# populationgenomics/cuKING

Measured on AMD Instinct MI355X. Metric: sample-pairs/s (all-pairs KING), higher is better.
Workload: dtype fp4 products, f32 accumulate (exact integers)

## Files before the change

### cuking_amd/csrc/king_abi.hip

```cpp
#include <hip/hip_runtime.h>

#include <algorithm>
#include <cstdio>
#include <cstdlib>
#include <cstring>
#include <vector>

#include "king_common.h"
#include "king_host.h"
#include "king_kin_summary.h"

using namespace cuking;

namespace {

#define HIP_TRY(expr)                                                      \
  do {                                                                     \
    const hipError_t _e = (expr);                                          \
    if (_e != hipSuccess) {                                                \
      (void)hipGetLastError();  \
      return cuking_fail(_e == hipErrorOutOfMemory ? CUKING_ERR_OUT_OF_MEMORY     \
                                            : CUKING_ERR_DEVICE,           \
                  "%s failed: %s", #expr, hipGetErrorString(_e));          \
    }                                                                      \
// ... 47 lines not shown
  }
};

}

struct cuking_ctx {
  int device = 0;
  cuking_kernel kernel = CUKING_KERNEL_TILED;
  int variant = 0;
  uint32_t band_rows = 0;
  int counts_mode = -1;
  int xcd_swizzle = 2;
  uint32_t dyn_tail_tiles = 16384;

  uint4 *planes = nullptr;
  size_t planes_bytes = 0;
  uint64_t *band_prefix = nullptr;
  size_t band_prefix_bytes = 0;
  TileSpace prefix_for = {0, 0, 0, 0};

  uint32_t split_wgs = 0;
  struct StreamScratch {
    hipStream_t stream;
    uint32_t *split = nullptr;
    uint8_t *filter = nullptr;
    uint64_t filter_tiles = 0;
  };
  std::vector<StreamScratch> scratch;
  unsigned long long filter_totals_retired[kNumTotals] = {};
  uint32_t filter_quadrant_cap = kFilterQuadrantCap;
  uint32_t filter_cand_cap = kFilterCandCap;
  uint32_t filter_split_min_steps = 8;
  int filter_check0 = 1, filter_check1 = 1, filter_check_emit = (int)kCheckEmitCap;
  int filter_rotate = 1;
  uint32_t filter_rotate_min_steps = 128;
  uint32_t filter_rotate_min_tiles = 2048;
  int filter_sort = 1;
  bool filter_lazy_codes = true;
  void *sort_temp = nullptr;
  size_t sort_temp_bytes = 0;

  void *synth_tables = nullptr;
  size_t synth_tables_bytes = 0;
  hipStream_t synth_stream = nullptr;
  hipEvent_t synth_done = nullptr;

  struct Prepared {
    bool valid = false;
    cuking_submatrix sm = {0, 0, 0, 0};
    uint32_t words_per_sample = 0;
    int variant = -1;
    uint32_t tile = 0;
    const uint64_t *bits = nullptr;
    bool codes = true;
    bool dense_order = false;
    std::vector<uint8_t> tiles;
    hipStream_t ordered_on = nullptr;
    bool ordered_valid = false;
  } prepared;
  std::vector<std::pair<hipStream_t, hipEvent_t>> readers;

  bool reuse_prepared = false;
  uint64_t workspace_allocations = 0, host_syncs = 0, conversions_skipped = 0;

  bool timing = false;
  Timer king_timer, prepare_timer;
// ... 142 lines not shown
                       mfma_split_scratch_bytes(ctx->split_wgs), 0,
                       mfma_split_counter_bytes(ctx->split_wgs), stream);
    if (st != CUKING_OK) return st;
  }
  const FilterScratchLayout want = filter_scratch_layout(tiles);
  if (filter && e->filter != nullptr && filter_scratch_layout(e->filter_tiles).bytes < want.bytes) {
    ++ctx->host_syncs;
    HIP_TRY(hipStreamSynchronize(stream));
    free_filter_scratch(ctx, *e);
  }
  if (filter && e->filter == nullptr) {
    st = alloc_scratch(ctx, reinterpret_cast<void **>(&e->filter), want.bytes, want.totals,
                       kFilterCtrlBytes + kFilterTicketBytes, stream);
    if (st != CUKING_OK) return st;
    e->filter_tiles = tiles;
  }
  *out = e;
  return CUKING_OK;
}

bool filter_runs(const cuking_ctx *ctx, uint32_t words_per_sample, bool full, float kin_threshold) {
  return effective_variant(ctx, words_per_sample) == kMfmaFilterVariant && !full &&
         kin_threshold > 0.f && kin_threshold < 0.5f;
}

LaunchSwitches launch_switches(const cuking_ctx *ctx, uint32_t words_per_sample, bool full,
                               float kin_threshold) {
  LaunchSwitches sw;
  sw.xcd_swizzle = (uint32_t)ctx->xcd_swizzle;
  sw.dyn_tail_tiles = ctx->dyn_tail_tiles;
  sw.check0 = (uint32_t)ctx->filter_check0;
  sw.check1 = (uint32_t)ctx->filter_check1;
  sw.check_emit = (uint32_t)ctx->filter_check_emit;
  sw.rotate = (uint32_t)ctx->filter_rotate;
  sw.rotate_min_tiles = ctx->filter_rotate_min_tiles;
  sw.split_min_steps = ctx->filter_split_min_steps;
  sw.filter_runs = filter_runs(ctx, words_per_sample, full, kin_threshold);
  return sw;
}

struct Outputs {
  uint32_t max_results;
  cuking_result *results;
  uint32_t *result_index, *result_overflow;
  cuking_counts *counts;
  float *kin;
  uint64_t kin_ld;
  uint32_t kin_flags;
  uint64_t *sum_hist, *sum_best;
  cuking_kin_bins sum_bins;
  uint32_t *rel_counts;
  uint32_t rel_num;
  float rel_thr[CUKING_REL_THRESHOLDS_MAX];
};
cuking_status launch_args(cuking_ctx *ctx, hipStream_t stream, const cuking_submatrix &sm,
                          uint32_t words_per_sample, const uint64_t *d_bit_sets,
                          const PlaneGeometry &geo, const TileSpace &tiles,
                          uint64_t block_tiles, float kin_threshold, const Outputs &out,
                          TiledArgs *args) {
  TiledArgs &a = *args;
  a = {};
  a.planes = ctx->planes;
  a.geo = geo;
  a.tiles = tiles;
  a.band_prefix = ctx->band_prefix;
  a.i_begin = sm.i_begin;
// ... 358 lines not shown
  const char *key;
  int64_t lo, hi;
  const char *error;
  uint32_t error_arg;
  uint8_t effects;
  int64_t (*get)(const cuking_ctx *);
  void (*set)(cuking_ctx *, int64_t);
  int64_t hole = INT64_MIN;
};

#define CTX_FIELD(f)                                                     \
  [](const cuking_ctx *c) -> int64_t { return (int64_t)c->f; },          \
  [](cuking_ctx *c, int64_t v) { c->f = (decltype(c->f))v; }

const Option kOptions[] = {
    {"variant", 0, kNumTiledVariants - 1, "variant outside [0, %u)", kNumTiledVariants, 0,
     CTX_FIELD(variant)},
    {"band_rows", 0, 64, "band_rows outside [0, 64]", 0, 0, CTX_FIELD(band_rows)},
    {"counts_mode", -1, 1, "counts_mode outside [-1, 1]", 0, 0, CTX_FIELD(counts_mode)},
    {"split_wgs", 0, 4096, "split_wgs outside [0, 4096]", 0, kResizesSlabs, CTX_FIELD(split_wgs)},
    {"xcd_swizzle", 0, 2, "xcd_swizzle outside [0, 2]", 0, 0, CTX_FIELD(xcd_swizzle)},
    {"dyn_tail_tiles", 0, 0x7FFFFFFF, "dyn_tail_tiles outside [0, 2^31)", 0, 0,
     CTX_FIELD(dyn_tail_tiles)},
    {"reuse_prepared", 0, 1, "reuse_prepared outside [0, 1]", 0, 0, CTX_FIELD(reuse_prepared)},
    {"filter_sort", 0, 2, "filter_sort outside [0, 2]", 0, kInvalidatesLayout,
     CTX_FIELD(filter_sort)},
    {"filter_lazy_codes", 0, 1, "filter_lazy_codes outside [0, 1]", 0, kInvalidatesLayout,
     CTX_FIELD(filter_lazy_codes)},
    {"filter_check0", 0, 2, "filter_check0 outside [0, 2]", 0, 0, CTX_FIELD(filter_check0)},
    {"filter_check1", 0, 1 + kNumCheckShares, "filter_check1 outside {0, 1, 3 .. %u}",
     1 + kNumCheckShares, 0, CTX_FIELD(filter_check1), 2},
    {"filter_check_emit", 0, 255, "filter_check_emit outside [0, 255]", 0, 0,
     CTX_FIELD(filter_check_emit)},
    {"filter_rotate", 0, 2 + kNumPhases, "filter_rotate outside [0, %u]", 2 + kNumPhases, 0,
     CTX_FIELD(filter_rotate)},
    {"filter_rotate_min_steps", 1, 1 << 20, "filter_rotate_min_steps outside [1, 2^20]", 0, 0,
     CTX_FIELD(filter_rotate_min_steps)},
    {"filter_rotate_min_tiles", 0, 1 << 30, "filter_rotate_min_tiles outside [0, 2^30]", 0, 0,
     CTX_FIELD(filter_rotate_min_tiles)},
    {"filter_quadrant_cap", 0, 16384, "filter_quadrant_cap outside [0, 16384]", 0, 0,
     CTX_FIELD(filter_quadrant_cap)},
    {"filter_cand_cap", 0, kFilterCandCap, "filter_cand_cap outside [0, %u]", kFilterCandCap, 0,
     CTX_FIELD(filter_cand_cap)},
    {"filter_split_min_steps", 1, 4096, "filter_split_min_steps outside [1, 4096]", 0, 0,
     CTX_FIELD(filter_split_min_steps)},
    {"max_launch_blocks", 0, INT64_MAX, "negative block cap", 0, 0,
     [](const cuking_ctx *) -> int64_t { return (int64_t)max_blocks_override(); },
     [](cuking_ctx *, int64_t v) { set_max_blocks_per_launch((uint64_t)v); }},
    {"filter_check_min_steps", 4, 1 << 20, "filter_check_min_steps outside [4, 2^20]", 0,
     kInvalidatesLayout,
     [](const cuking_ctx *) -> int64_t { return filter_check_min_steps(); },
     [](cuking_ctx *, int64_t v) { set_filter_check_min_steps((uint32_t)v); }},
};
#undef CTX_FIELD

const Option *find_option(const char *key) {
  for (const Option &o : kOptions)
    if (strcmp(o.key, key) == 0) return &o;
  return nullptr;
}

cuking_status read_diagnostic(const cuking_ctx *ctx, const char *key, int64_t *value) {
  const std::pair<const char *, uint64_t> counters[] = {
      {"workspace_allocations", ctx->workspace_allocations},
      {"host_syncs", ctx->host_syncs},
      {"conversions_skipped", ctx->conversions_skipped}};
  for (const auto &c : counters)
    if (strcmp(c.first, key) == 0) {
      *value = (int64_t)c.second;
      return CUKING_OK;
    }
  const char *const totals[kNumTotals] = {"filter_candidates", "filter_dense_quadrants",
                                          "filter_early_exits", "filter_rotated_tiles"};
  static_assert(kTotalCand == 0 && kTotalDense == 1 && kTotalEarly == 2 && kTotalRotated == 3,
                "totals[] in the order of the running totals");
  uint32_t word = 0;
  while (word < kNumTotals && strcmp(totals[word], key) != 0) ++word;
  const bool ticks = strcmp(key, "filter_step_ticks16") == 0;
  if (word == kNumTotals && !ticks)
    return cuking_fail(CUKING_ERR_INVALID_ARGUMENT, "unknown option %s", key);
  if (hipSetDevice(ctx->device) != hipSuccess || hipDeviceSynchronize() != hipSuccess)
    return cuking_fail(CUKING_ERR_DEVICE, "device wait failed");
  unsigned long long sum = 0;
  uint64_t count = 0;
  for (const auto &e : ctx->scratch) {
    if (e.filter == nullptr) continue;
    if (ticks) {
      uint32_t w[8];
      if (hipMemcpy(w, e.filter + kCtrlStepTicks * 4, sizeof w, hipMemcpyDeviceToHost) != hipSuccess)
        return cuking_fail(CUKING_ERR_DEVICE, "reading the filter counters failed");
      for (uint32_t v : w)
        if (v != 0) {
          sum += v;
          ++count;
        }
    } else {
      unsigned long long v = 0;
      if (hipMemcpy(&v, e.filter + filter_scratch_layout(e.filter_tiles).totals + word * 8, 8,
                    hipMemcpyDeviceToHost) != hipSuccess)
        return cuking_fail(CUKING_ERR_DEVICE, "reading the filter counters failed");
      sum += v;
    }
  }
  if (ticks) *value = count != 0 ? (int64_t)(sum / count) : 0;
  else *value = (int64_t)(sum + ctx->filter_totals_retired[word]);
  return CUKING_OK;
}
// ... 877 lines not shown
```

### cuking_amd/csrc/king_common.h

```cpp
#ifndef CUKING_AMD_KING_COMMON_H_
#define CUKING_AMD_KING_COMMON_H_

#include <hip/hip_runtime.h>
#include <stdint.h>

#include "cuking_amd.h"
#include "king_launch_plan.h"
#include "king_submatrix.h"

namespace cuking {

constexpr uint32_t kLayoutWord = 0;
constexpr uint32_t kLayoutQuad = 1;
constexpr uint32_t kLayoutNibble = 2;
constexpr uint32_t kLayoutNibbleStats = 3;

struct PlaneGeometry {
  uint32_t num_rows, num_cols;
  uint32_t rows_padded, cols_padded;
  uint32_t col_base;
  uint32_t s_stride;
  uint32_t k_words;
  uint32_t diag;
};
// ... 76 lines not shown
  uint32_t dense_cap;
  uint32_t fsplit_parts, fsplit_first, fsplit_tile0;
  float4 *fsplit_slabs;
  uint32_t *fsplit_tickets;
  const uint32_t *check_steps;
  const float *prefix_u;
  const unsigned long long *cohort_sums;
  uint32_t check0, check1;
  uint32_t rotate, rotate_min_steps;
  uint32_t rotate_min_tiles;
  uint8_t *tile_done;
  const uint32_t *gate;
  uint32_t gate_count;
  const uint8_t *skip_tiles;
  uint64_t skip_base;
  const uint32_t *perm;
  uint32_t *codes_ready;
  float *dense_kin;
  uint64_t kin_ld;
  uint32_t kin_diag;
  unsigned long long *sum_hist, *sum_best;
  float sum_lo, sum_scale;
  uint32_t sum_bins;
  uint32_t *rel_counts;
  uint32_t rel_num;
  float rel_thr[CUKING_REL_THRESHOLDS_MAX];
};

constexpr uint32_t kCheckEmitCap = 64;
constexpr uint32_t kNumCheckShares = 8;
constexpr uint32_t kCheckShares64[kNumCheckShares] = {8, 50, 53, 56, 58, 60, 61, 62};
constexpr uint32_t kNumPhases = 128;
constexpr uint32_t kPhasesPerShare = kNumPhases / 64;
constexpr uint32_t kNumCum = kNumPhases - 1;
__host__ __device__ inline uint32_t phase_step(uint32_t all_steps, uint32_t x) {
  return (uint32_t)((uint64_t)all_steps * x / kNumPhases);
}
__host__ __device__ inline uint32_t check_step_of(uint32_t all_steps, uint32_t k,
                                                  uint32_t min_steps = 64) {
  if (all_steps < min_steps) return 0;
  return phase_step(all_steps, kCheckShares64[k] * kPhasesPerShare);
}
constexpr uint32_t kFilterSplitSlabs = 256;
constexpr size_t kFilterSlabBytes = 256 * 256 * sizeof(float);
constexpr size_t kFilterTicketBytes = kFilterSplitSlabs * sizeof(uint32_t);
__host__ __device__ inline size_t plane_bytes(const PlaneGeometry &g,
                                              uint32_t layout) {
  const size_t base = (size_t)g.k_words * g.s_stride * (layout == kLayoutQuad ? 8 : 16);
  if (layout == kLayoutNibble) return base + base / 4;
  if (layout == kLayoutNibbleStats)
    return base + base / 4 + base / 2 + (size_t)g.s_stride * sizeof(float2) +
           (size_t)g.s_stride * kNumCum * sizeof(float) + 64 + 64 +
           64 + (size_t)g.s_stride * (4 + 8 + 4 * (kNumCum + 1) + 16);
  return base;
}
__host__ __device__ inline const uint4 *plane_t2(const uint4 *planes, const PlaneGeometry &g) {
  return planes + (size_t)g.k_words * g.s_stride * 5 / 4;
}
__host__ __device__ inline const float2 *plane_stats(const uint4 *planes, const PlaneGeometry &g) {
  return reinterpret_cast<const float2 *>(planes + (size_t)g.k_words * g.s_stride * 7 / 4);
}
__host__ __device__ inline const float *plane_prefix_u(const uint4 *planes, const PlaneGeometry &g) {
  return reinterpret_cast<const float *>(plane_stats(planes, g) + g.s_stride);
}
__host__ __device__ inline const unsigned long long *plane_cohort_sums(const uint4 *planes,
                                                                       const PlaneGeometry &g) {
  return reinterpret_cast<const unsigned long long *>(plane_prefix_u(planes, g) +
                                                      (size_t)g.s_stride * kNumCum);
}

struct TiledVariant {
  const char *name;
  uint32_t tile;
  uint32_t k_chunk;
  uint32_t threads;
  uint32_t lds_bytes;
  uint32_t layout;
};

constexpr uint32_t kMfmaMaxSites = 1u << 24;

constexpr int kNumTiledVariants = 8;
constexpr int kMfmaVariant = 5;
constexpr int kMfmaN4Variant = 6;
constexpr uint32_t kMfmaN4MaxSites = 1u << 22;
static_assert(4ull * kMfmaN4MaxSites <= (1ull << 24), "filter kernel: exact float sums");
constexpr int kMfmaN4Stages = 5;
constexpr uint32_t kMfmaN4LdsBytes = kMfmaN4Stages * 2 * 2 * 4 * 128 * 16;
static_assert(kMfmaN4LdsBytes <= 160 * 1024, "LDS of one CU");
constexpr int kMfmaFilterVariant = 7;
constexpr uint32_t kFilterTile = 256;
constexpr uint32_t kFilterLdsBytes = 5 * 2 * 2 * 2 * 256 * 16;
static_assert(kFilterLdsBytes <= 160 * 1024, "LDS of one CU");
constexpr uint32_t kFilterChunkTiles = 1u << 17;
constexpr uint32_t kFilterCandCap = 1u << 25;
constexpr uint32_t kFilterQuadrantCap = 384;
constexpr size_t kFilterCtrlBytes = 256;
constexpr uint32_t kCtrlCand = 0, kCtrlDense = 1, kCtrlDyn = 2, kCtrlFinished = 3,
                   kCtrlLeft = 4, kCtrlAllLeave = 5, kCtrlGate = 6;
constexpr uint32_t kCtrlStepTicks = 8, kCtrlPos = 16, kPosSlots = 16;
constexpr size_t kCtrlChunkBytes = (kCtrlPos + 8 * kPosSlots * 2) * 4;
constexpr uint32_t kTotalCand = 0, kTotalDense = 1, kTotalEarly = 2, kTotalRotated = 3;
constexpr uint32_t kNumTotals = 4;
__host__ __device__ inline const uint32_t *plane_check_steps(const uint4 *planes,
                                                             const PlaneGeometry &g) {
  return reinterpret_cast<const uint32_t *>(plane_cohort_sums(planes, g) + 8);
}
__host__ __device__ inline uint32_t *plane_flags(const uint4 *planes, const PlaneGeometry &g) {
  return const_cast<uint32_t *>(plane_check_steps(planes, g)) + 16;
}
__host__ __device__ inline uint32_t *plane_perm(const uint4 *planes, const PlaneGeometry &g) {
  return plane_flags(planes, g) + 16;
}
__host__ __device__ inline float2 *plane_tmp_stats(const uint4 *planes, const PlaneGeometry &g) {
  return reinterpret_cast<float2 *>(plane_perm(planes, g) + g.s_stride);
}
__host__ __device__ inline float *plane_tmp_prefix(const uint4 *planes, const PlaneGeometry &g) {
  return reinterpret_cast<float *>(plane_tmp_stats(planes, g) + g.s_stride);
}
__host__ __device__ inline uint32_t *plane_sort_words(const uint4 *planes, const PlaneGeometry &g) {
  return reinterpret_cast<uint32_t *>(plane_tmp_prefix(planes, g) +
                                      (size_t)g.s_stride * (kNumCum + 1));
}
constexpr uint32_t kNoSample = 0xFFFFFFFFu;

struct FilterScratchLayout {
  size_t tile_done, totals, tickets, cand, dense, slabs, bytes;
  uint32_t chunk_tiles, cand_entries;
};
inline FilterScratchLayout filter_scratch_layout(uint64_t tiles) {
  FilterScratchLayout l;
  l.chunk_tiles = (uint32_t)(tiles < kFilterChunkTiles ? (tiles ? tiles : 1) : kFilterChunkTiles);
  const uint64_t cand = (uint64_t)l.chunk_tiles * 4 * 64;
  l.cand_entries = (uint32_t)(cand < kFilterCandCap ? cand : kFilterCandCap);
  auto up = [](size_t x) { return (x + 255) / 256 * 256; };
  l.tile_done = kCtrlChunkBytes;
// ... 98 lines not shown
```

### cuking_amd/csrc/king_filter.hip

```cpp
#include <hip/hip_runtime.h>
#include <stdio.h>

#include <atomic>
#include <stdlib.h>

#include "king_common.h"
#include "king_device.h"
#include "king_kin_summary.h"

#pragma clang diagnostic ignored "-Winline-asm"

namespace cuking {

namespace {

typedef int v8i __attribute__((ext_vector_type(8)));
typedef float v16f __attribute__((ext_vector_type(16)));

constexpr int kT = (int)kFilterTile;
constexpr int kUnits = 2;
constexpr int kStages = 5;
constexpr int kSliceU4 = kT;
constexpr int kStageU4 = 2 * 2 * kUnits * kSliceU4;
constexpr int kStageReqs = 4 * kUnits;
// ... 143 lines not shown
  if (a.dyn_tiles != 0 && wg >= a.launch_tiles) {
    uint32_t *slot = reinterpret_cast<uint32_t *>(lds);
    if (threadIdx.x == 0) *slot = relaxed_add(a.filter_ctrl + kCtrlDyn, 1u);
    __syncthreads();
    const uint32_t next = __builtin_amdgcn_readfirstlane(*slot);
    __syncthreads();
    if (next >= a.dyn_tiles) return false;
    bid = a.launch_tiles + next;
  } else if (a.xcd_chunk == 1) {
    bid = xcd_patch_tile(bid);
    if (bid >= a.launch_tiles) return false;
  }
  t->bid = __builtin_amdgcn_readfirstlane(bid);
  uint32_t tr, tc;
  if (!decode_tile_space(a, a.tile_begin + t->bid, &tr, &tc)) return false;
  t->tr = __builtin_amdgcn_readfirstlane(tr);
  t->tc = __builtin_amdgcn_readfirstlane(tc);
  return true;
}

__device__ __forceinline__ bool launch_verdict(const TiledArgs &a, const uint32_t wg,
                                               uint4 *const lds, uint32_t *xcd_pos) {
  uint32_t *verdict = reinterpret_cast<uint32_t *>(lds);
  if (threadIdx.x == 0) {
    uint32_t leave = relaxed_load(a.filter_ctrl + kCtrlAllLeave);
    auto all_leave = [&] {
      leave = 1;
      relaxed_store(a.filter_ctrl + kCtrlAllLeave, 1u);
      relaxed_store(a.filter_ctrl + kCtrlGate, 1u);
    };
    float mean, sigma;
    if (leave == 0 && a.cohort_sums != nullptr && a.check_steps != nullptr &&
        bound_level(a.cohort_sums, 32.f * (float)a.geo.k_words, &mean, &sigma) &&
        mean - 4.f * sigma > a.kin_threshold && (a.check1 >> 16) != 0)
      all_leave();
    if (leave == 0) {
      const uint32_t dense_so_far =
          relaxed_load(a.filter_ctrl + kCtrlDense) + relaxed_load(a.filter_ctrl + kCtrlLeft);
      const uint32_t finished = relaxed_load(a.filter_ctrl + kCtrlFinished);
      if (finished >= 512 && 2 * dense_so_far > finished) all_leave();
    }
    verdict[0] = leave;
  }
  if (a.rotate == 1 && threadIdx.x < kPosSlots) {
    const uint32_t x = wg & 7;
    const unsigned long long said = relaxed_load(
        reinterpret_cast<const unsigned long long *>(a.filter_ctrl + kCtrlPos) + x * kPosSlots +
        threadIdx.x);
    const uint32_t ticks16 = relaxed_load(a.filter_ctrl + kCtrlStepTicks + x);
    uint32_t pos = (uint32_t)(said >> 32);
    const uint32_t ago = (uint32_t)__builtin_amdgcn_s_memrealtime() - (uint32_t)said;
    if (said != 0 && ticks16 != 0 && ago < 16384u)
      pos += ago * 16u / ticks16;
    verdict[1 + threadIdx.x] = pos;
  }
  __syncthreads();
  const bool give_up = verdict[0] != 0;
  uint32_t pos = 0;
  if (a.rotate == 1) {
#pragma unroll
    for (uint32_t k = 0; k < kPosSlots; ++k) pos = max(pos, verdict[1 + k]);
  }
  *xcd_pos = __builtin_amdgcn_readfirstlane(pos);
  __syncthreads();
  if (give_up && threadIdx.x == 0) relaxed_add(a.filter_totals + kTotalDense, 4ull);
  return give_up;
}

struct CheckPlan {
  uint32_t chk0, chk1;
  uint32_t share1;
  uint32_t phase;
  uint32_t k0;
  uint32_t wrap;
  uint32_t start_abs;
};
__device__ __forceinline__ CheckPlan plan_checks(const TiledArgs &a, const Tile &t,
                                                 const uint32_t xcd_pos, const uint32_t all_steps,
                                                 const uint32_t num_steps) {
  uint32_t chk0 = 0, chk1 = 0, entry1 = 0, share1 = 0;
  uint32_t phase = 0, k0 = 0, wrap = 0, start_abs = 0;
  if (!t.split && a.check_steps != nullptr && a.tile_done != nullptr) {
    if (a.rotate != 0 && all_steps >= a.rotate_min_steps) {
      uint32_t base = 0;
      if (a.rotate == 1) {
        const uint32_t r = xcd_pos % all_steps;
        base = xcd_pos - r;
        phase = (r * kNumPhases + all_steps / 2) / all_steps;
        if (phase >= kNumPhases) {
          phase = 0;
          base += all_steps;
        }
      } else if (a.rotate == 2) {
        phase = (t.bid * 37u + 11u) & (kNumPhases - 1);
      } else {
        phase = (a.rotate - 3u) & (kNumPhases - 1);
      }
      k0 = phase_step(all_steps, phase);
      start_abs = base + k0;
      wrap = k0 != 0 ? all_steps - k0 : 0u;
    }
    float kappa = -1.f, mean, sigma;
    if (bound_level(a.cohort_sums, 256.f * (float)all_steps, &mean, &sigma))
      kappa = mean + 4.6f * sigma + 0.003f;
    auto steps_of = [&](uint32_t share) {
      const uint32_t hi = phase + share * kPhasesPerShare;
      return hi <= kNumPhases ? phase_step(all_steps, hi) - k0
                              : (all_steps - k0) + phase_step(all_steps, hi - kNumPhases);
    };
    if ((a.check0 == 2 || (a.check0 == 1 && kappa > 0.7f * a.kin_threshold)) &&
        a.check_steps[0] != 0)
      chk0 = steps_of(kCheckShares64[0]);
    const uint32_t sw1 = a.check1 & 0xFFu;
    if (sw1 >= 2) {
      entry1 = sw1 - 2;
    } else if (sw1 == 1 && kappa >= 0.f) {
      const float f64 = 64.f * (1.f - 2.f * a.kin_threshold) / (1.f - 2.f * kappa);
      if (f64 <= 62.f) {
        share1 = (uint32_t)ceilf(f64);
        if (share1 < 32) share1 = 32;
        entry1 = 1;
      }
    }
#pragma unroll
    for (uint32_t k = 1; k < kNumCheckShares; ++k)
      if (sw1 >= 2 && k == entry1) share1 = kCheckShares64[k];
    if (share1 != 0 && a.check_steps[entry1] != 0) chk1 = steps_of(share1);
    if (chk0 >= num_steps) chk0 = 0;
    if (chk1 >= num_steps || chk1 <= chk0) chk1 = 0;
  }
  auto sgpr = [](uint32_t v) { return (uint32_t)__builtin_amdgcn_readfirstlane(v); };
  return CheckPlan{sgpr(chk0), sgpr(chk1), sgpr(share1), sgpr(phase), sgpr(k0), sgpr(wrap), sgpr(start_abs)};
}

__device__ __forceinline__ float prefix_u_of(const TiledArgs &a, const CheckPlan &p,
                                             uint32_t share, size_t idx, float total) {
  const uint32_t s_stride = a.geo.s_stride;
  const uint32_t hi = p.phase + share * kPhasesPerShare;
  float u = hi >= kNumPhases ? total
            : hi != 0        ? a.prefix_u[(size_t)(hi - 1) * s_stride + idx]
                             : 0.f;
  if (p.phase != 0) u -= a.prefix_u[(size_t)(p.phase - 1) * s_stride + idx];
  if (hi > kNumPhases) u += a.prefix_u[(size_t)(hi - kNumPhases - 1) * s_stride + idx];
  return u;
}

__device__ __forceinline__ const float2 *stage_bounds(const TiledArgs &a, const Tile &t,
                                                      const CheckPlan &p, uint4 *const lds,
                                                      const bool prefix, const uint32_t share,
                                                      const float thr, const float scale) {
  float2 *const rows = reinterpret_cast<float2 *>(lds), *const cols = rows + kT;
  const float tt = 2.f - 4.f * thr;
  const size_t ir = (size_t)t.tr * kT + threadIdx.x;
  const size_t ic = (size_t)a.geo.col_base + (size_t)t.tc * kT + threadIdx.x;
  float2 r = a.sample_stats[ir], c = a.sample_stats[ic];
  if (prefix) {
    r.x = prefix_u_of(a, p, share, ir, r.x);
    c.x = prefix_u_of(a, p, share, ic, c.x);
  }
  r.y = scale * fmaf(tt, r.y, 8.f);
  c.y = scale * fmaf(tt, c.y, 8.f);
  rows[threadIdx.x] = r;
  cols[threadIdx.x] = c;
  __syncthreads();
  return rows;
}

enum Leave : uint32_t { kStays = 0, kLeftForecast, kLeftEmpty, kLeftEmit };

__device__ __forceinline__ Leave check_sweep(const TiledArgs &a, const Tile &t, const CheckPlan &p,
                                             const v16f (&acc)[4][4], uint4 *const lds,
                                             const bool forecast, const uint32_t all_steps) {
  const Lanes l = lanes_of_thread();
  const float scale = forecast ? (float)kCheckShares64[0] * (1.f / 64.f) : 1.f;
  const uint32_t share = forecast ? kCheckShares64[0] : p.share1;
  const float thr_f = forecast ? a.kin_threshold + 3.66f * rsqrtf(256.f * (float)all_steps)
                               : a.kin_threshold;
  const float2 *const ck_rows = stage_bounds(a, t, p, lds, true, share, thr_f, scale);
  const float2 *const ck_cols = ck_rows + kT;
  uint32_t *const ck_words = reinterpret_cast<uint32_t *>(lds) + 4 * kT;
  const uint32_t emit_cap = (a.check1 >> 8) & 0xFFu;
  uint32_t cnt = 0;
  {
    float2 cc[4];
#pragma unroll
    for (int bj = 0; bj < 4; ++bj) cc[bj] = ck_cols[l.wx * 128 + bj * 32 + l.lr];
#pragma unroll
    for (int bi = 0; bi < 4; ++bi)
#pragma unroll
      for (int r = 0; r < 16; ++r) {
        const float2 cr = ck_rows[l.wy * 128 + bi * 32 + c_row(r, l.g)];
#pragma unroll
        for (int bj = 0; bj < 4; ++bj)
          cnt += fmaf(-8.f, acc[bi][bj][r], cr.x) + cc[bj].x < fminf(cr.y, cc[bj].y) ? 1u : 0u;
      }
  }
#pragma unroll
  for (int off = 32; off > 0; off >>= 1) cnt += __shfl_xor(cnt, off);
  if (l.lane == 0)
    ck_words[l.wave] = forecast ? (cnt > 2 * a.quadrant_cap ? 1u : 0u)
                                : (cnt > emit_cap ? emit_cap + 1 : cnt);
  __syncthreads();
  uint32_t found = forecast ? ck_words[0] + ck_words[1] + ck_words[2] + ck_words[3]
                            : max(max(ck_words[0], ck_words[1]), max(ck_words[2], ck_words[3]));
  found = __builtin_amdgcn_readfirstlane(found);
  __syncthreads();
  if (forecast) return found >= 3 ? kLeftForecast : kStays;
  return found > emit_cap ? kStays : found != 0 ? kLeftEmit : kLeftEmpty;
}

__device__ __forceinline__ bool leave_early(const TiledArgs &a, const Tile &t, const CheckPlan &p,
                                            const Leave left) {
  if (left == kLeftEmit && threadIdx.x == 0) relaxed_add(a.filter_totals + kTotalEarly, 1ull);
  if (p.phase != 0 && threadIdx.x == 0) relaxed_add(a.filter_totals + kTotalRotated, 1ull);
  if (left == kLeftForecast || left == kLeftEmpty) {
    if (threadIdx.x == 0) {
      relaxed_add(a.filter_ctrl + kCtrlFinished, 4u);
      if (left == kLeftForecast) {
        relaxed_add(a.filter_ctrl + kCtrlLeft, 4u);
        relaxed_store(a.filter_ctrl + kCtrlGate, 1u);
        relaxed_add(a.filter_totals + kTotalDense, 4ull);
      } else {
        a.tile_done[t.bid] = 1;
        relaxed_add(a.filter_totals + kTotalEarly, 1ull);
      }
    }
    return true;
  }
  if (!t.split && a.tile_done != nullptr && threadIdx.x == 0) a.tile_done[t.bid] = 1;
  return false;
}

__device__ __forceinline__ bool reduce_pieces(const TiledArgs &a, const Tile &t, v16f (&acc)[4][4],
                                              uint4 *const lds) {
  typedef uint32_t v4u __attribute__((ext_vector_type(4)));
  constexpr uint32_t kSlabU4 = 64 * 256;
  {
    const __amdgpu_buffer_rsrc_t rsrc = __builtin_amdgcn_make_buffer_rsrc(
        a.fsplit_slabs + (size_t)t.piece * kSlabU4, 0, (int)(kSlabU4 * 16), 0x00020000);
#pragma unroll
    for (int bi = 0; bi < 4; ++bi)
#pragma unroll
      for (int bj = 0; bj < 4; ++bj)
#pragma unroll
        for (int r4 = 0; r4 < 4; ++r4) {
          const v16f &c = acc[bi][bj];
// ... 14 lines not shown
    if (last) {
      __builtin_amdgcn_fence(__ATOMIC_ACQUIRE, "agent");
      asm volatile("s_waitcnt vmcnt(0)" ::: "memory");
      *counter = 0;
    }
    *flag = last ? 1u : 0u;
  }
  __syncthreads();
  const bool last = *flag != 0;
  __syncthreads();
  if (!last) return false;
  const uint32_t first_piece = t.piece - t.part;
  for (uint32_t p = 0; p < a.fsplit_parts; ++p) {
    if (p == t.part) continue;
    const float4 *src = a.fsplit_slabs + (size_t)(first_piece + p) * kSlabU4 + threadIdx.x;
#pragma unroll
    for (int bi = 0; bi < 4; ++bi)
#pragma unroll
      for (int bj = 0; bj < 4; ++bj)
#pragma unroll
        for (int r4 = 0; r4 < 4; ++r4) {
          const float4 v = src[((bi * 4 + bj) * 4 + r4) * 256];
          acc[bi][bj][4 * r4] += v.x;
          acc[bi][bj][4 * r4 + 1] += v.y;
          acc[bi][bj][4 * r4 + 2] += v.z;
          acc[bi][bj][4 * r4 + 3] += v.w;
        }
  }
  return true;
}

__device__ __forceinline__ void emit_candidates(const TiledArgs &a, const Tile &t,
                                                const CheckPlan &p, const v16f (&acc)[4][4],
                                                uint4 *const lds, const bool on_prefix) {
  const Lanes l = lanes_of_thread();
  const float2 *const st_rows = stage_bounds(a, t, p, lds, on_prefix, p.share1, a.kin_threshold, 1.f);
  const float2 *const st_cols = st_rows + kT;
  float2 sc[4];
#pragma unroll
  for (int bj = 0; bj < 4; ++bj) sc[bj] = st_cols[l.wx * 128 + bj * 32 + l.lr];

  {
    float best = -1.f;
#pragma unroll
    for (int bi = 0; bi < 4; ++bi)
#pragma unroll
      for (int r = 0; r < 16; ++r) {
        const float2 sr = st_rows[l.wy * 128 + bi * 32 + c_row(r, l.g)];
#pragma unroll
        for (int bj = 0; bj < 4; ++bj)
          best = fmaxf(best, fminf(sr.y, sc[bj].y) -
                                 (fmaf(-8.f, acc[bi][bj][r], sr.x) + sc[bj].x));
      }
    if (l.lane == 0) relaxed_add(a.filter_ctrl + kCtrlFinished, 1u);
    if (__ballot(best > 0.f) == 0) return;
  }

  uint32_t total = 0, base = 0, run = 0;
#pragma nounroll
  for (int pass = 0; pass < 2; ++pass) {
    uint32_t tr_p = t.tr, tc_p = t.tc;
    asm volatile("" : "+s"(tr_p), "+s"(tc_p));
#pragma unroll
    for (int bi = 0; bi < 4; ++bi) {
#pragma unroll
      for (int r = 0; r < 16; ++r) {
        const uint32_t row = l.wy * 128 + bi * 32 + c_row(r, l.g);
        const float2 sr = st_rows[row];
        const uint32_t li = tr_p * kT + row;
// ... 158 lines not shown
    const uint32_t t16_ = (STEPS) >= 32 ? (now_ - t_start) * 16u / (STEPS) : 0u; \
    const uint32_t zero_ = 0;                                                  \
    unsigned long long save_;                                                  \
    asm volatile("s_mov_b64 %0, exec\n\t"                                      \
                 "s_mov_b64 exec, 1\n\t"                                       \
                 "global_store_dwordx2 %1, %2, %3\n\t"                         \
                 "s_mov_b64 exec, %0"                                          \
                 : "=&s"(save_)                                                \
                 : "v"(zero_), "v"(val_), "s"(pos_word)                        \
                 : "memory");                                                  \
    if (t16_ != 0)                                                             \
      asm volatile("s_mov_b64 %0, exec\n\t"                                    \
                   "s_mov_b64 exec, 1\n\t"                                     \
                   "global_store_dword %1, %2, %3\n\t"                         \
                   "s_mov_b64 exec, %0"                                        \
                   : "=&s"(save_)                                              \
                   : "v"(zero_), "v"(t16_), "s"(ticks_word)                    \
                   : "memory");                                                \
  }

__device__ __forceinline__ void filter_tile(const TiledArgs &a, const uint32_t wg, uint4 *const lds) {
  Tile tile;
  if (!take_tile(a, wg, lds, &tile)) return;
  const Lanes ln = lanes_of_thread();
  uint32_t xcd_pos = 0;
  if (!tile.split && a.tile_done != nullptr && launch_verdict(a, wg, lds, &xcd_pos)) return;
  const uint32_t all_steps = a.geo.k_words / (4 * kUnits);
  const uint32_t k_first = __builtin_amdgcn_readfirstlane(
      tile.split ? tile.part * all_steps / a.fsplit_parts : 0u);
  const uint32_t num_steps = __builtin_amdgcn_readfirstlane(
      tile.split ? (tile.part + 1) * all_steps / a.fsplit_parts - k_first : all_steps);
  const CheckPlan plan = plan_checks(a, tile, xcd_pos, all_steps, num_steps);

  const uint32_t wave = ln.wave, chk0 = plan.chk0, chk1 = plan.chk1;
  const uint32_t k0 = plan.k0, wrap = plan.wrap, start_abs = plan.start_abs;
  uint32_t lane16 = ln.lane * 16;
  const uint32_t s_stride = a.geo.s_stride;
  const uint4 *g_rows = a.t2 + (uint64_t)tile.tr * kT;
  const uint4 *g_cols = a.t2 + a.geo.col_base + (uint64_t)tile.tc * kT;

  uint32_t mT, mA;
  asm volatile("s_mov_b32 %0, 0xcccccccc" : "=s"(mT));
  asm volatile("s_mov_b32 %0, 0x33333333" : "=s"(mA));
  int scaleB;
  asm volatile("v_mov_b32 %0, 0x7d7d7d7d" : "=v"(scaleB));

  const uint32_t dma_side = wave >> 1, dma_h = wave & 1;
  const uint32_t row_bytes = s_stride * 16;
  const char *const g_wave = reinterpret_cast<const char *>(
      (dma_side ? g_cols : g_rows) + ((uint64_t)2 * kUnits * k_first + kUnits * dma_h) * s_stride);
  const uint32_t l_wave = (uint32_t)(uintptr_t)(lds_void_ptr)(
      lds + ((dma_side * 2 + dma_h) * kUnits) * kSliceU4);
  struct Addr { const char *src; uint32_t dst; };
  const uint32_t kstep_bytes = 2 * kUnits * row_bytes;
  const char *seg_src = g_wave;
  uint32_t seg_steps = num_steps;
  uint32_t seg_wrap = 0xFFFFFFFFu;
  auto addr_of = [&](uint32_t step, uint32_t buf) {
    Addr pa;
    if (step >= seg_steps) step = seg_steps - 1;
    const int32_t rel = (int32_t)step - (int32_t)(step >= seg_wrap ? all_steps : 0u);
    pa.src = seg_src + (int64_t)rel * (int64_t)kstep_bytes;
    pa.dst = l_wave + buf * (kStageU4 * 16);
    asm volatile("" : "+s"(pa.src), "+s"(pa.dst));
    return pa;
  };
  auto addr_next = [&](const Addr &cur, uint32_t step, uint32_t buf) {
    Addr pa;
    const int32_t adv = (int32_t)(step < seg_steps ? 1u : 0u) -
                        (int32_t)(step == seg_wrap ? all_steps : 0u);
    pa.src = cur.src + (int64_t)adv * (int64_t)kstep_bytes;
    pa.dst = l_wave + buf * (kStageU4 * 16);
    asm volatile("" : "+s"(pa.src), "+s"(pa.dst));
    return pa;
  };

  v16f acc[4][4] = {};

  uint32_t row_off = ((0 * 2 + ln.g) * kUnits) * kSliceU4 + ln.wy * 128 + ln.lr;
  uint32_t col_off = ((1 * 2 + ln.g) * kUnits) * kSliceU4 + ln.wx * 128 + ln.lr;
  asm volatile("" : "+v"(row_off), "+v"(col_off), "+v"(lane16));
  v8i FA[2][4], FB[2][4];
  uint4 RAW[8];

  unsigned long long *const pos_word =
      reinterpret_cast<unsigned long long *>(a.filter_ctrl + kCtrlPos) +
      (wg & 7) * kPosSlots + ((wg >> 3) & (kPosSlots - 1));
  uint32_t *const ticks_word = a.filter_ctrl + kCtrlStepTicks + (wg & 7);
  const uint32_t t_start = a.rotate == 1 ? (uint32_t)__builtin_amdgcn_s_memrealtime() : 0u;

  uint32_t seg_first = 0;
  Leave left = kStays;
#pragma nounroll
  while (true) {
    uint32_t seg_end = num_steps;
    if (chk1 > seg_first) seg_end = chk1;
    if (chk0 > seg_first) seg_end = chk0;
    seg_end = __builtin_amdgcn_readfirstlane(seg_end);
    seg_steps = seg_end - seg_first;
    const uint32_t seg_k = seg_first >= wrap && wrap != 0 ? seg_first - wrap : k0 + seg_first;
    seg_src = g_wave + (uint64_t)seg_k * kstep_bytes;
    seg_wrap = __builtin_amdgcn_readfirstlane(
        wrap > seg_first && wrap < seg_end ? wrap - seg_first : 0xFFFFFFFFu);
    asm volatile("" : "+s"(seg_src), "+s"(seg_steps), "+s"(seg_wrap));

#pragma unroll
    for (int st = 0; st < kStages - 1; ++st) {
      const Addr p0 = addr_of(st, st);
      F_ISSUE4(p0, 0)
      F_ISSUE4(p0, 1)
    }
    __builtin_amdgcn_s_waitcnt(vmcnt_imm((kStages - 2) * kStageReqs));
    __syncthreads();
#pragma unroll
    for (int k = 0; k < 8; ++k) {
      F_READ(k, 0, 0)
    }
#pragma unroll
    for (int k = 0; k < 8; ++k) {
      F_BUILD_B(0, k)
    }
    uint32_t buf = 0;
    Addr pa = addr_of(kStages - 1, kStages - 1);
    uint32_t step = 0;
    while (step + 1 < seg_steps) {
      F_KSTEP
      F_KSTEP
    }
    if (step < seg_steps) F_KSTEP
    __builtin_amdgcn_s_waitcnt(0x0F70);
    __syncthreads();
    F_PUBLISH(seg_end)
    if (seg_end == num_steps) break;

    left = check_sweep(a, tile, plan, acc, lds, seg_end == chk0, all_steps);
    if (left != kStays) break;
    seg_first = seg_end;
  }

  if (leave_early(a, tile, plan, left)) return;
  if (tile.split && !reduce_pieces(a, tile, acc, lds)) return;
  emit_candidates(a, tile, plan, acc, lds, left == kLeftEmit);
}
#undef F_KSTEP
#undef F_SLICE_A
#undef F_SLICE_B
#undef F_BAR
#undef F_MMA
#undef F_BUILD_A
#undef F_BUILD_B
#undef F_PIN4
#undef F_PINF
#undef F_READ
#undef F_ISSUE4
#undef F_ISSUE
#undef F_PUBLISH

__global__ __launch_bounds__(256, 1) void king_filter_kernel(const TiledArgs a) {
  extern __shared__ uint4 lds[];
  filter_tile(a, blockIdx.x, lds);
}

__global__ __launch_bounds__(256) void king_refine_kernel(const TiledArgs a) {
  const uint32_t lane = threadIdx.x & 63;
  uint32_t count = *a.filter_ctrl;
  if (count > a.cand_cap) count = a.cand_cap;
  const uint32_t n = a.words_per_sample / 2;
  const uint32_t stride = gridDim.x * 4;
  for (uint32_t p = blockIdx.x * 4 + (threadIdx.x >> 6); p < count; p += stride) {
    const uint2 e = a.cand_list[p];
    if (e.x == kNoPair) continue;
    const uint32_t off_i = a.perm != nullptr ? a.perm[e.x] : e.x;
    const uint32_t off_j = a.perm != nullptr ? a.perm[a.geo.col_base + e.y]
                                             : (a.geo.diag ? e.y : a.geo.num_rows + e.y);
    const uint64_t *het_i_w = a.bits + (uint64_t)off_i * a.words_per_sample;
// ... 202 lines not shown
```

### cuking_amd/csrc/king_launch_plan.h

```cpp
#ifndef CUKING_AMD_KING_LAUNCH_PLAN_H_
#define CUKING_AMD_KING_LAUNCH_PLAN_H_

#include <stdint.h>

namespace cuking {

struct LaunchSwitches {
  uint32_t xcd_swizzle, dyn_tail_tiles;
  uint32_t check0, check1, check_emit, rotate, rotate_min_tiles, split_min_steps;
  bool filter_runs;
};

struct WholeShape {
  uint64_t tiles;
  uint32_t launch_tiles, xcd_chunk, dyn_tiles, dyn_wgs;
  uint64_t grid;
};

inline WholeShape whole_shape(uint64_t want, uint64_t cap, uint32_t xcd_swizzle, uint64_t dyn_min,
                              uint64_t dyn_floor) {
  const bool xcd_order = xcd_swizzle != 0 && cap >= 64;
  if (xcd_order) cap &= ~7ull;
  uint64_t n = want < cap ? want : cap;
  WholeShape s = {};
  uint64_t dyn = 0, dyn_wgs = 0;
  if (dyn_min != 0 && xcd_swizzle == 2 && xcd_order && n >= dyn_min && n >= dyn_floor) {
    if (n + n / 8 > cap) n = cap - cap / 8;
    const uint64_t fixed = (n - n / 16) / 256 * 256;
    dyn = n - fixed;
    dyn_wgs = dyn + dyn / 2;
    if (fixed + dyn_wgs > cap) dyn = dyn_wgs = 0;
  }
  s.tiles = n;
  s.dyn_tiles = (uint32_t)dyn;
  s.dyn_wgs = (uint32_t)dyn_wgs;
  s.launch_tiles = (uint32_t)(n - dyn);
  s.grid = n;
  if (dyn != 0) {
    s.xcd_chunk = 1;
    s.grid = n - dyn + dyn_wgs;
  } else if (xcd_order && n >= 64) {
    if (xcd_swizzle == 2) {
      const uint64_t patches = (n + 31) / 32;
// ... 31 lines not shown
inline MfmaPlan mfma_plan(uint64_t num_tiles, uint32_t wgs, uint32_t tile_steps, uint64_t cap) {
  constexpr uint64_t kSplitRounds = 64;
  uint32_t rest = 0;
  if (wgs != 0 && num_tiles < kSplitRounds * wgs) {
    rest = num_tiles < 2ull * wgs ? (uint32_t)num_tiles : (uint32_t)(num_tiles % wgs);
    if ((uint64_t)rest * tile_steps < 8ull * wgs) rest = 0;
  }
  if (rest == 0) return {num_tiles, 0, 0};
  const uint64_t head = num_tiles - rest;
  uint64_t first = 0;
  if (cap <= wgs + wgs / 2) {
    first = head;
  } else if (head + wgs + wgs / 2 > cap) {
    first = head + wgs + wgs / 2 - cap;
  }
  return {first, (uint32_t)(head - first), rest};
}

struct FilterPlan {
  uint64_t n;
  uint32_t check0, check1, rotate;
  uint32_t rest, parts;
  WholeShape whole;
  uint32_t fsplit_tile0, fsplit_first;
  uint64_t grid;
};
inline FilterPlan filter_plan(uint64_t want, uint64_t cap, uint32_t wgs, uint32_t tile_steps,
                              bool checks, bool can_split, uint32_t max_slabs,
                              const LaunchSwitches &sw) {
  FilterPlan p = {};
  const uint64_t n = want < cap ? want : cap;
  p.n = n;
  p.check0 = !checks ? 0u : sw.check0 == 2 ? 2u : (sw.check0 == 1 && n < 16ull * wgs) ? 1u : 0u;
  p.check1 = checks ? sw.check1 | (sw.check_emit << 8) | (sw.check0 != 0 ? 1u << 16 : 0u) : 0u;
  p.rotate = checks && (n >= sw.rotate_min_tiles || sw.rotate >= 2) ? sw.rotate : 0u;
  uint32_t rest = 0, parts = 0;
  if (can_split && n < 16ull * wgs) {
    rest = (uint32_t)(n % wgs);
    if (rest != 0 && 2 * rest <= wgs && rest <= max_slabs / 2) {
      parts = wgs / rest;
      if (parts > 8) parts = 8;
      if (parts * rest > max_slabs) parts = max_slabs / rest;
      const uint32_t min_steps = sw.split_min_steps != 0 ? sw.split_min_steps : 8;
      while (parts > 1 && tile_steps / parts < min_steps) --parts;
    }
    if (parts < 2) rest = parts = 0;
  }
  p.rest = rest;
  p.parts = parts;
  p.whole = whole_shape(n - rest, ~0ull, sw.xcd_swizzle == 2 ? 2u : 0u,
                        filter_dyn_min(sw.dyn_tail_tiles), kFilterDynFloor);
  p.fsplit_tile0 = (uint32_t)(n - rest);
  p.fsplit_first = (uint32_t)p.whole.grid;
  p.grid = p.whole.grid + (uint64_t)rest * parts;
  return p;
}

}

#endif
```

Measured before the change: 38.18 billion.

## Add a second early-exit check phase to the KING filter kernel

Adds an optional second mid-loop check (chk2), placed a few phases after the first check, so tiles whose candidates are already settled can leave the MFMA k-loop sooner. Check shares are now expressed in 128-phase units instead of 64-share units, and the kappa margin is retuned. The second check is enabled by default through a new filter_check2 option packed into the check1 word, and a new running total counts exits at the second check. The cost is an extra bounds sweep per tile that reaches chk2, which is wasted work for tiles that do not exit there.

```diff
diff --git a/cuking_amd/csrc/king_abi.hip b/cuking_amd/csrc/king_abi.hip
--- a/cuking_amd/csrc/king_abi.hip
+++ b/cuking_amd/csrc/king_abi.hip
@@ -103,6 +103,7 @@
   uint32_t filter_cand_cap = kFilterCandCap;
   uint32_t filter_split_min_steps = 8;
   int filter_check0 = 1, filter_check1 = 1, filter_check_emit = (int)kCheckEmitCap;
+  int filter_check2 = 1;
   int filter_rotate = 1;
   uint32_t filter_rotate_min_steps = 128;
   uint32_t filter_rotate_min_tiles = 2048;
@@ -311,6 +312,7 @@
   sw.check0 = (uint32_t)ctx->filter_check0;
   sw.check1 = (uint32_t)ctx->filter_check1;
   sw.check_emit = (uint32_t)ctx->filter_check_emit;
+  sw.check2 = (uint32_t)ctx->filter_check2;
   sw.rotate = (uint32_t)ctx->filter_rotate;
   sw.rotate_min_tiles = ctx->filter_rotate_min_tiles;
   sw.split_min_steps = ctx->filter_split_min_steps;
@@ -735,6 +737,8 @@
      1 + kNumCheckShares, 0, CTX_FIELD(filter_check1), 2},
     {"filter_check_emit", 0, 255, "filter_check_emit outside [0, 255]", 0, 0,
      CTX_FIELD(filter_check_emit)},
+    {"filter_check2", 0, 2 + kCheck2MaxForced, "filter_check2 outside {0, 1, 3 .. %u}",
+     2 + kCheck2MaxForced, 0, CTX_FIELD(filter_check2), 2},
     {"filter_rotate", 0, 2 + kNumPhases, "filter_rotate outside [0, %u]", 2 + kNumPhases, 0,
      CTX_FIELD(filter_rotate)},
     {"filter_rotate_min_steps", 1, 1 << 20, "filter_rotate_min_steps outside [1, 2^20]", 0, 0,
@@ -774,8 +778,10 @@
       return CUKING_OK;
     }
   const char *const totals[kNumTotals] = {"filter_candidates", "filter_dense_quadrants",
-                                          "filter_early_exits", "filter_rotated_tiles"};
-  static_assert(kTotalCand == 0 && kTotalDense == 1 && kTotalEarly == 2 && kTotalRotated == 3,
+                                          "filter_early_exits", "filter_rotated_tiles",
+                                          "filter_early_exits2"};
+  static_assert(kTotalCand == 0 && kTotalDense == 1 && kTotalEarly == 2 && kTotalRotated == 3 &&
+                    kTotalEarly2 == 4,
                 "totals[] in the order of the running totals");
   uint32_t word = 0;
   while (word < kNumTotals && strcmp(totals[word], key) != 0) ++word;
diff --git a/cuking_amd/csrc/king_common.h b/cuking_amd/csrc/king_common.h
--- a/cuking_amd/csrc/king_common.h
+++ b/cuking_amd/csrc/king_common.h
@@ -132,6 +132,9 @@
 constexpr uint32_t kCheckShares64[kNumCheckShares] = {8, 50, 53, 56, 58, 60, 61, 62};
 constexpr uint32_t kNumPhases = 128;
 constexpr uint32_t kPhasesPerShare = kNumPhases / 64;
+constexpr uint32_t kCheckMinPhases = 32 * kPhasesPerShare, kCheckMaxPhases = 62 * kPhasesPerShare;
+constexpr uint32_t kCheck2Phases = 4, kCheck2MinRest = 8, kCheck2MaxForced = 63;
+constexpr float kCheckLiveBudget = 0.1f, kCheckBudgetZ = 4.67f;
 constexpr uint32_t kNumCum = kNumPhases - 1;
 __host__ __device__ inline uint32_t phase_step(uint32_t all_steps, uint32_t x) {
   return (uint32_t)((uint64_t)all_steps * x / kNumPhases);
@@ -194,14 +197,17 @@
 static_assert(kFilterLdsBytes <= 160 * 1024, "LDS of one CU");
 constexpr uint32_t kFilterChunkTiles = 1u << 17;
 constexpr uint32_t kFilterCandCap = 1u << 25;
+static_assert(kCheckLiveBudget * 1024.f <= 256.f, "check budget against the candidate list");
 constexpr uint32_t kFilterQuadrantCap = 384;
 constexpr size_t kFilterCtrlBytes = 256;
 constexpr uint32_t kCtrlCand = 0, kCtrlDense = 1, kCtrlDyn = 2, kCtrlFinished = 3,
                    kCtrlLeft = 4, kCtrlAllLeave = 5, kCtrlGate = 6;
 constexpr uint32_t kCtrlStepTicks = 8, kCtrlPos = 16, kPosSlots = 16;
 constexpr size_t kCtrlChunkBytes = (kCtrlPos + 8 * kPosSlots * 2) * 4;
-constexpr uint32_t kTotalCand = 0, kTotalDense = 1, kTotalEarly = 2, kTotalRotated = 3;
-constexpr uint32_t kNumTotals = 4;
+constexpr uint32_t kTotalCand = 0, kTotalDense = 1, kTotalEarly = 2, kTotalRotated = 3,
+                   kTotalEarly2 = 4;
+constexpr uint32_t kNumTotals = 5;
+static_assert(kNumTotals * 8 <= kFilterCtrlBytes, "the running totals have kFilterCtrlBytes");
 __host__ __device__ inline const uint32_t *plane_check_steps(const uint4 *planes,
                                                              const PlaneGeometry &g) {
   return reinterpret_cast<const uint32_t *>(plane_cohort_sums(planes, g) + 8);
diff --git a/cuking_amd/csrc/king_filter.hip b/cuking_amd/csrc/king_filter.hip
--- a/cuking_amd/csrc/king_filter.hip
+++ b/cuking_amd/csrc/king_filter.hip
@@ -199,7 +199,7 @@
     float mean, sigma;
     if (leave == 0 && a.cohort_sums != nullptr && a.check_steps != nullptr &&
         bound_level(a.cohort_sums, 32.f * (float)a.geo.k_words, &mean, &sigma) &&
-        mean - 4.f * sigma > a.kin_threshold && (a.check1 >> 16) != 0)
+        mean - 4.f * sigma > a.kin_threshold && ((a.check1 >> 16) & 1u) != 0)
       all_leave();
     if (leave == 0) {
       const uint32_t dense_so_far =
@@ -236,7 +236,9 @@
 
 struct CheckPlan {
   uint32_t chk0, chk1;
+  uint32_t chk2;
   uint32_t share1;
+  uint32_t share2;
   uint32_t phase;
   uint32_t k0;
   uint32_t wrap;
@@ -245,7 +247,7 @@
 __device__ __forceinline__ CheckPlan plan_checks(const TiledArgs &a, const Tile &t,
                                                  const uint32_t xcd_pos, const uint32_t all_steps,
                                                  const uint32_t num_steps) {
-  uint32_t chk0 = 0, chk1 = 0, entry1 = 0, share1 = 0;
+  uint32_t chk0 = 0, chk1 = 0, chk2 = 0, entry1 = 0, share1 = 0, share2 = 0;
   uint32_t phase = 0, k0 = 0, wrap = 0, start_abs = 0;
   if (!t.split && a.check_steps != nullptr && a.tile_done != nullptr) {
     if (a.rotate != 0 && all_steps >= a.rotate_min_steps) {
@@ -269,41 +271,51 @@
     }
     float kappa = -1.f, mean, sigma;
     if (bound_level(a.cohort_sums, 256.f * (float)all_steps, &mean, &sigma))
-      kappa = mean + 4.6f * sigma + 0.003f;
+      kappa = mean + kCheckBudgetZ * sigma;
     auto steps_of = [&](uint32_t share) {
-      const uint32_t hi = phase + share * kPhasesPerShare;
+      const uint32_t hi = phase + share;
       return hi <= kNumPhases ? phase_step(all_steps, hi) - k0
                               : (all_steps - k0) + phase_step(all_steps, hi - kNumPhases);
     };
     if ((a.check0 == 2 || (a.check0 == 1 && kappa > 0.7f * a.kin_threshold)) &&
         a.check_steps[0] != 0)
-      chk0 = steps_of(kCheckShares64[0]);
+      chk0 = steps_of(kCheckShares64[0] * kPhasesPerShare);
     const uint32_t sw1 = a.check1 & 0xFFu;
     if (sw1 >= 2) {
       entry1 = sw1 - 2;
     } else if (sw1 == 1 && kappa >= 0.f) {
-      const float f64 = 64.f * (1.f - 2.f * a.kin_threshold) / (1.f - 2.f * kappa);
-      if (f64 <= 62.f) {
-        share1 = (uint32_t)ceilf(f64);
-        if (share1 < 32) share1 = 32;
+      const float f128 =
+          (float)kNumPhases * (1.f - 2.f * a.kin_threshold) / (1.f - 2.f * kappa);
+      if (f128 <= (float)kCheckMaxPhases) {
+        share1 = (uint32_t)ceilf(f128);
+        if (share1 < kCheckMinPhases) share1 = kCheckMinPhases;
         entry1 = 1;
       }
     }
 #pragma unroll
     for (uint32_t k = 1; k < kNumCheckShares; ++k)
-      if (sw1 >= 2 && k == entry1) share1 = kCheckShares64[k];
+      if (sw1 >= 2 && k == entry1) share1 = kCheckShares64[k] * kPhasesPerShare;
     if (share1 != 0 && a.check_steps[entry1] != 0) chk1 = steps_of(share1);
     if (chk0 >= num_steps) chk0 = 0;
     if (chk1 >= num_steps || chk1 <= chk0) chk1 = 0;
+    const uint32_t sw2 = a.check1 >> 24;
+    if (chk1 != 0 && sw2 != 0) {
+      share2 = share1 + (sw2 >= 2 ? sw2 - 2 : kCheck2Phases);
+      if (share2 < kNumPhases && (sw2 >= 2 || share2 + kCheck2MinRest <= kNumPhases))
+        chk2 = steps_of(share2);
+      if (chk2 >= num_steps || chk2 <= chk1) chk2 = 0;
+    }
+    if (chk2 == 0) share2 = 0;
   }
   auto sgpr = [](uint32_t v) { return (uint32_t)__builtin_amdgcn_readfirstlane(v); };
-  return CheckPlan{sgpr(chk0), sgpr(chk1), sgpr(share1), sgpr(phase), sgpr(k0), sgpr(wrap), sgpr(start_abs)};
+  return CheckPlan{sgpr(chk0),  sgpr(chk1), sgpr(chk2), sgpr(share1), sgpr(share2),
+                   sgpr(phase), sgpr(k0),   sgpr(wrap), sgpr(start_abs)};
 }
 
 __device__ __forceinline__ float prefix_u_of(const TiledArgs &a, const CheckPlan &p,
                                              uint32_t share, size_t idx, float total) {
   const uint32_t s_stride = a.geo.s_stride;
-  const uint32_t hi = p.phase + share * kPhasesPerShare;
+  const uint32_t hi = p.phase + share;
   float u = hi >= kNumPhases ? total
             : hi != 0        ? a.prefix_u[(size_t)(hi - 1) * s_stride + idx]
                              : 0.f;
@@ -337,10 +349,10 @@
 
 __device__ __forceinline__ Leave check_sweep(const TiledArgs &a, const Tile &t, const CheckPlan &p,
                                              const v16f (&acc)[4][4], uint4 *const lds,
-                                             const bool forecast, const uint32_t all_steps) {
+                                             const bool forecast, const uint32_t share,
+                                             const uint32_t all_steps) {
   const Lanes l = lanes_of_thread();
-  const float scale = forecast ? (float)kCheckShares64[0] * (1.f / 64.f) : 1.f;
-  const uint32_t share = forecast ? kCheckShares64[0] : p.share1;
+  const float scale = forecast ? (float)share * (1.f / (float)kNumPhases) : 1.f;
   const float thr_f = forecast ? a.kin_threshold + 3.66f * rsqrtf(256.f * (float)all_steps)
                                : a.kin_threshold;
   const float2 *const ck_rows = stage_bounds(a, t, p, lds, true, share, thr_f, scale);
@@ -377,8 +389,10 @@
 }
 
 __device__ __forceinline__ bool leave_early(const TiledArgs &a, const Tile &t, const CheckPlan &p,
-                                            const Leave left) {
+                                            const Leave left, const bool second) {
   if (left == kLeftEmit && threadIdx.x == 0) relaxed_add(a.filter_totals + kTotalEarly, 1ull);
+  if ((left == kLeftEmit || left == kLeftEmpty) && second && threadIdx.x == 0)
+    relaxed_add(a.filter_totals + kTotalEarly2, 1ull);
   if (p.phase != 0 && threadIdx.x == 0) relaxed_add(a.filter_totals + kTotalRotated, 1ull);
   if (left == kLeftForecast || left == kLeftEmpty) {
     if (threadIdx.x == 0) {
@@ -459,9 +473,10 @@
 
 __device__ __forceinline__ void emit_candidates(const TiledArgs &a, const Tile &t,
                                                 const CheckPlan &p, const v16f (&acc)[4][4],
-                                                uint4 *const lds, const bool on_prefix) {
+                                                uint4 *const lds, const bool on_prefix,
+                                                const uint32_t share) {
   const Lanes l = lanes_of_thread();
-  const float2 *const st_rows = stage_bounds(a, t, p, lds, on_prefix, p.share1, a.kin_threshold, 1.f);
+  const float2 *const st_rows = stage_bounds(a, t, p, lds, on_prefix, share, a.kin_threshold, 1.f);
   const float2 *const st_cols = st_rows + kT;
   float2 sc[4];
 #pragma unroll
@@ -686,7 +701,7 @@
       tile.split ? (tile.part + 1) * all_steps / a.fsplit_parts - k_first : all_steps);
   const CheckPlan plan = plan_checks(a, tile, xcd_pos, all_steps, num_steps);
 
-  const uint32_t wave = ln.wave, chk0 = plan.chk0, chk1 = plan.chk1;
+  const uint32_t wave = ln.wave, chk0 = plan.chk0, chk1 = plan.chk1, chk2 = plan.chk2;
   const uint32_t k0 = plan.k0, wrap = plan.wrap, start_abs = plan.start_abs;
   uint32_t lane16 = ln.lane * 16;
   const uint32_t s_stride = a.geo.s_stride;
@@ -744,10 +759,12 @@
   const uint32_t t_start = a.rotate == 1 ? (uint32_t)__builtin_amdgcn_s_memrealtime() : 0u;
 
   uint32_t seg_first = 0;
+  uint32_t seg_share = 0;
   Leave left = kStays;
 #pragma nounroll
   while (true) {
     uint32_t seg_end = num_steps;
+    if (chk2 > seg_first) seg_end = chk2;
     if (chk1 > seg_first) seg_end = chk1;
     if (chk0 > seg_first) seg_end = chk0;
     seg_end = __builtin_amdgcn_readfirstlane(seg_end);
@@ -787,14 +804,18 @@
     F_PUBLISH(seg_end)
     if (seg_end == num_steps) break;
 
-    left = check_sweep(a, tile, plan, acc, lds, seg_end == chk0, all_steps);
+    seg_share = __builtin_amdgcn_readfirstlane(
+        seg_end == chk0   ? kCheckShares64[0] * kPhasesPerShare
+        : seg_end == chk1 ? plan.share1
+                          : plan.share2);
+    left = check_sweep(a, tile, plan, acc, lds, seg_end == chk0, seg_share, all_steps);
     if (left != kStays) break;
     seg_first = seg_end;
   }
 
-  if (leave_early(a, tile, plan, left)) return;
+  if (leave_early(a, tile, plan, left, seg_share == plan.share2)) return;
   if (tile.split && !reduce_pieces(a, tile, acc, lds)) return;
-  emit_candidates(a, tile, plan, acc, lds, left == kLeftEmit);
+  emit_candidates(a, tile, plan, acc, lds, left == kLeftEmit, seg_share);
 }
 #undef F_KSTEP
 #undef F_SLICE_A
diff --git a/cuking_amd/csrc/king_launch_plan.h b/cuking_amd/csrc/king_launch_plan.h
--- a/cuking_amd/csrc/king_launch_plan.h
+++ b/cuking_amd/csrc/king_launch_plan.h
@@ -9,6 +9,7 @@
   uint32_t xcd_swizzle, dyn_tail_tiles;
   uint32_t check0, check1, check_emit, rotate, rotate_min_tiles, split_min_steps;
   bool filter_runs;
+  uint32_t check2;
 };
 
 struct WholeShape {
@@ -106,7 +107,9 @@
   const uint64_t n = want < cap ? want : cap;
   p.n = n;
   p.check0 = !checks ? 0u : sw.check0 == 2 ? 2u : (sw.check0 == 1 && n < 16ull * wgs) ? 1u : 0u;
-  p.check1 = checks ? sw.check1 | (sw.check_emit << 8) | (sw.check0 != 0 ? 1u << 16 : 0u) : 0u;
+  p.check1 = checks ? sw.check1 | (sw.check_emit << 8) | (sw.check0 != 0 ? 1u << 16 : 0u) |
+                          (sw.check2 << 24)
+                    : 0u;
   p.rotate = checks && (n >= sw.rotate_min_tiles || sw.rotate >= 2) ? sw.rotate : 0u;
   uint32_t rest = 0, parts = 0;
   if (can_split && n < 16ull * wgs) {
```

Result: no change. 38.48 billion (median of 6 runs) (+0.8%).
